# EPFL-IMOS/simple-SFOD

Measured on AMD Instinct MI355X. Metric: teacher+student train images/s on 1024x2048 synthetic, higher is better.
Workload: dtype bf16x3

## Files before the change

include/sfod_hip.h:

```cpp
#ifndef SFOD_HIP_H
#define SFOD_HIP_H
#include <stdint.h>
#ifdef __cplusplus
extern "C" {
#endif

#define SFOD_F32 0
#define SFOD_BF16 1
#define SFOD_BF16X3 2
#define SFOD_F16X3 3

int sfod_version(void);
const char* sfod_last_error(void);

int sfod_preprocess(const void* const* img_ptrs, const int32_t* sizes, int B, int Hp, int Wp,
                    int Cpad, const float* mean3, const float* std3, void* out, int dt,
                    void* stream);

int sfod_hflip_u8(const void* src, void* dst, int C, int H, int W, void* stream);

int sfod_resize_bilinear_u8(const void* src, void* dst, int C, int H, int W, int h, int w,
                            const int32_t* hbounds, const int32_t* hcoef, int ksize_h,
                            const int32_t* vbounds, const int32_t* vcoef, int ksize_v, int flip,
                            void* stream);
int sfod_resize_bilinear_u8_opt(const void* src, void* dst, int C, int H, int W, int y0, int x0, int ch, int cw,
                                int h, int w, const int32_t* hbounds, const int32_t* hcoef, int ksize_h,
                                const int32_t* vbounds, const int32_t* vcoef, int ksize_v, int flip_mode,
                                void* stream);

int sfod_mosaic_u8(const void* const* tiles, const void* const* tabs, const int32_t* geom, int n_tiles, int fill,
                   void* out, int H0, int W0, void* stream);

int sfod_conv_fwd(const void* x, const void* w, const float* bias, void* y, int B, int H, int W,
                  int Cin, int Cout, int ksize, int ldy, int act, float* stats, int dt, int out_dt,
                  void* stream);
int sfod_conv_fwd_ws(const void* x, const void* w, const uint32_t* w_absmax, const float* bias, void* y, int B, int H,
                     int W, int Cin, int Cout, int ksize, int ldy, int act, float* stats, int dt, int out_dt,
                     void* stream);
int64_t sfod_conv_fwd_scratch_bytes(int B, int H, int W, int Cin, int Cout, int ksize, int dt, int out_dt, int with_stats);
int sfod_conv_fwd_scratch(const void* x, const void* w, const uint32_t* w_absmax, const float* bias, void* y, int B, int H,
                          int W, int Cin, int Cout, int ksize, int ldy, int act, float* stats, int dt, int out_dt,
                          void* scratch, int64_t scratch_bytes, void* stream);
int sfod_conv_stats_blocks(int B, int H, int W, int Cin, int Cout, int ksize, int dt);
int sfod_set_conv_algo(int algo);
int sfod_conv_dgrad_bnred_blocks(int B, int H, int W, int Cin, int Cout, int dt);
int sfod_conv_dgrad_bnred(const void* x, const void* w, void* dz, int B, int H, int W, int Cin, int Cout, int dt,
                          const float* y, const float* mean, const float* invstd, const float* gamma,
                          const float* beta, float* red_ws, void* stream);
int sfod_conv_fwd_bnin_supported(int B, int H, int W, int Cin, int Cout, int dt);
int sfod_conv_fwd_bnin(const float* x_pre, const float* in_mean, const float* in_invstd, const float* in_gamma,
                       const float* in_beta, const void* w, const float* bias, float* y, int B, int H, int W, int Cin,
                       int Cout, int ldy, int act, float* stats, int dt, void* stream);
int sfod_set_gemm_tile(int tile);
int sfod_set_conv3x3_variant(int variant);
int sfod_last_conv_kernel(char* buf, int n);
int sfod_set_deterministic(int on);
int sfod_get_deterministic(void);
int sfod_set_conv3x3_m16(int on);
int sfod_set_wgrad3x3_pipe(int on);
int sfod_conv_fwd_algo(int B, int H, int W, int Cin, int Cout, int ksize, int dt);

int sfod_conv_first_supported(int B, int H, int W, int Cin, int Cout, int dt, int ldy);
int sfod_conv_first_fused(const void* x, const void* w, const float* bias, const float* scale,
                          const float* shift, void* y, float* stats, int B, int H, int W, int ldy,
                          int act, int dt, void* stream);
int sfod_conv_first_fused_ws(const void* x, const void* w, const uint32_t* w_absmax, const float* bias,
                             const float* scale, const float* shift, void* y, float* stats, int B, int H, int W,
                             int ldy, int act, int dt, void* stream);
int sfod_conv_first_stats_blocks(int B, int H, int W);
int sfod_set_conv_first_pipe(int on);
int sfod_set_conv_first_grid(int n);
int sfod_conv_first_bn_apply_supported(int B, int H, int W, int Cin, int Cout, int pool_flags, int dt, int y_dt);
int sfod_conv_first_bn_apply(const void* x, const void* w, const float* bias, const float* mean, const float* invstd,
                             const float* gamma, const float* beta, void* z, int B, int H, int W, int ldz, int dt,
                             void* stream);
int sfod_set_first_apply_recompute(int on);

int64_t sfod_conv_wgrad_ws_bytes(int B, int H, int W, int Cin, int Cout, int ksize, int lddy, int dt);
int sfod_conv_wgrad(const void* x, const void* dy, float* dw, int B, int H, int W, int Cin,
                    int Cout, int ksize, int lddy, int dt, void* ws, int64_t ws_bytes, void* stream);
int sfod_conv_wgrad_oihw_supported(int B, int H, int W, int Cin, int Cout, int ksize, int lddy, int dt);
int sfod_conv_wgrad_oihw(const void* x, const void* dy, float* dw_oihw, int B, int H, int W, int Cin,
                         int Cout, int ksize, int lddy, int dt, int accumulate, void* ws,
                         int64_t ws_bytes, void* stream);
int sfod_conv_first_wgrad_bn_supported(int B, int H, int W, int Cin, int Cout, int pool, int dt, int y_dt);
int sfod_conv_first_wgrad_bn(const void* x, const void* dz, const void* y, const float* mean, const float* invstd,
                             const float* gamma, const float* beta, const float* dgamma, const float* dbeta,
                             float* dw, int B, int H, int W, int Cin, int Cout, int dt, int oihw, int accumulate,
                             void* ws, int64_t ws_bytes, void* stream);
int sfod_set_first_wgrad_fused(int on);

int sfod_pack_conv_weight(const float* w_oihw, void* w_packed, int Cout, int Cin, int ksize,
                          int CinPad, int rot180, int dt, void* stream);
int sfod_pack_conv_weight_ws(const float* w_oihw, void* w_packed, uint32_t* absmax, int Cout, int Cin, int ksize,
                             int CinPad, int rot180, int dt, void* stream);
int sfod_pack_conv_weights_blocks(int Cout, int Cin, int ksize, int innerPad, int rot180);
int sfod_pack_conv_weights_multi(const int64_t* desc, int n, int total_blocks, int dt, void* stream);
int sfod_pack_conv_weights_multi_ws(const int64_t* desc, int n, int total_blocks, int dt, uint32_t* absmax ,
                                    void* stream);
int sfod_unpack_conv_wgrad(const float* dw_packed, float* dw_oihw, int Cout, int Cin, int ksize,
                           int CinPad, int accumulate, void* stream);
int sfod_pack_fc_weight(const float* w, void* out, int N, int K, int chw_c, int transpose, int dt,
                        void* stream);
int sfod_unpack_fc_wgrad(const float* dw_packed, float* dw, int N, int K, int chw_c,
                         int accumulate, void* stream);
int sfod_pack_fc_weight_ld(const float* w, void* out, int N, int K, int chw_c, int transpose, int ld,
                           int dt, void* stream);
int sfod_pack_fc_weight_ld_ws(const float* w, void* out, uint32_t* absmax, int N, int K, int chw_c, int transpose,
                              int ld, int dt, void* stream);
int sfod_unpack_fc_wgrad_ld(const float* dw_packed, float* dw, int N, int K, int chw_c, int ld,
                            int accumulate, void* stream);
int sfod_bias_grad(const void* dy, float* db, int M, int N, int ld, int accumulate, int dt,
                   void* stream);

int sfod_bn_finalize(const float* stats, int nblocks, int M, int C,
                     float* mean, float* invstd, float* running_mean, float* running_var,
                     float momentum, float eps, int update_running, int64_t* num_batches_tracked,
                     float* ws, void* stream);
int sfod_bn_finalize_pop(const float* stats, int nblocks, int M, int C,
                         float* mean, float* invstd, float* running_mean, float* running_var,
                         float momentum, float eps, int update_running, int64_t* num_batches_tracked,
                         float* ws, double* pop, int64_t pop_stride, void* stream);
int sfod_bn_pop_commit(const double* pop, int64_t pop_stride, const int64_t* table, const int64_t* table_host, int n,
                       void* stream);
int sfod_bn_pop_merge(double* dst, const double* src, int64_t columns, void* stream);
int sfod_set_bn_finalize_fused(int on);
int sfod_bn_finalize_ws_floats(int C);
int sfod_bn_relu_pool_fwd(const void* y, const float* mean, const float* invstd,
                          const float* gamma, const float* beta, void* z, int B, int H, int W,
                          int C, int pool, int dt, int out_dt, void* stream);
int sfod_bn_relu_pool_fwd2(const void* y, const float* mean, const float* invstd,
                           const float* gamma, const float* beta, void* z, void* z2, int B, int H, int W,
                           int C, int pool, int dt, int out_dt, void* stream);
int sfod_bn_add_relu_fwd(const void* y, const float* mean, const float* invstd, const float* gamma,
                         const float* beta, const void* residual, void* z, void* z_pairs, void* z_pairs2, int64_t rows,
                         int C, int dt, int pairs_dt, void* stream);
int sfod_bn_relu_pool_bwd(const void* dz, const void* y, const float* mean, const float* invstd,
                          const float* gamma, const float* beta, void* dy, float* dgamma,
                          float* dbeta, float* dgamma_acc, float* dbeta_acc, float* ws, int B, int H,
                          int W, int C, int pool, int dt, int out_dt, int reduced_blocks, void* stream);
#define SFOD_BN_BWD_SCRATCH_ROWS 32
int sfod_bn_bwd_ws_floats(int M, int C);
// ... 218 lines not shown
```

simple-sfod_amd/csrc/conv_internal.h:

```cpp
#pragma once
#include "common.h"

struct P3Plan {
  int ok;
  int G;
  int FM;
  int TH, TW;
  int tiles_y, tiles_x, tiles_n;
  int nblk;
  int m16;
};
P3Plan sfod_p3_plan(int B, int H, int W, int Cin, int Cout, int pairs = 0);
struct P3BnRed {
  const float* y;
  const float* mean;
  const float* invstd;
  const float* gamma;
  const float* beta;
  float* ws;
};
struct P3BnIn {
  const float* mean;
  const float* invstd;
  const float* gamma;
  const float* beta;
};
bool sfod_p3_bnin_ok(const P3Plan& p, int Cin_phys, int split);
int sfod_p3_launch(const P3Plan& p, const void* x, const void* w, const float* bias, void* y, float* stats,
                   int B, int H, int W, int Cin, int Cout, int ldy, int act, int out_f32, hipStream_t s, int split = 0,
                   const P3BnRed* red = nullptr, const unsigned* wamax = nullptr, const P3BnIn* bnin = nullptr);


struct W3Plan {
  int ok;
  int CO;
  int TH, TW, tiles_y, tiles_x;
  int co_tiles, ci_tiles;
  int tiles_per_split, nsplit, nslab;
  int64_t ws_bytes;
  int w64;
};
W3Plan sfod_w3_plan(int B, int H, int W, int Cin, int Cout, int lddy, int split = 0);
int sfod_w3_launch(const W3Plan& p, const void* x, const void* dy, float* dw, void* ws, int B, int H, int W,
                   int Cin, int Cout, int lddy, int out_mode, hipStream_t s, int split = 0);

struct W3BnApply {
  const float* dz;
  const float* y;
  const float* mean;
  const float* invstd;
  const float* gamma;
  const float* beta;
  const float* dgamma;
  const float* dbeta;
};
bool sfod_w3_bn_ok(const W3Plan& p, int Cin, int Cout);
int sfod_w3_bn_launch(const W3Plan& p, const void* x, const W3BnApply& bn, float* dw, void* ws, int B, int H, int W,
                      int out_mode, hipStream_t s);

bool sfod_deterministic();

void sfod_f16_poll_elementwise(unsigned* out, hipStream_t s);
void sfod_f16_poll_roi(unsigned* out, hipStream_t s);
void sfod_f16_poll_first(unsigned* out, hipStream_t s);
void sfod_f16_poll_stem(unsigned* out, hipStream_t s);
void sfod_f16_poll_gn(unsigned* out, hipStream_t s);
void sfod_f16_poll_cda(unsigned* out, hipStream_t s);

int sfod_f1_nblk(int B, int H, int W);
bool sfod_f1_bn_ok(int W);
struct F1BnApply {
  const float* mean;
  const float* invstd;
  const float* gamma;
  const float* beta;
};
int sfod_f1_launch(const void* x, const void* w, const float* bias, void* y, float* stats, int B, int H, int W,
                   int ldy, int act, hipStream_t s, const float* scale = nullptr, const float* shift = nullptr, int split = 0,
                   const unsigned* wamax = nullptr, const F1BnApply* bn = nullptr);
```

simple-sfod_amd/csrc/gemm_conv.hip:

```cpp
#include "conv_internal.h"
#include <algorithm>

typedef __attribute__((ext_vector_type(8))) __bf16 bf16x8;
typedef __attribute__((ext_vector_type(4))) short s16x4;
typedef __attribute__((ext_vector_type(8))) short s16x8;
typedef __attribute__((ext_vector_type(16))) float f32x16;
typedef __attribute__((ext_vector_type(4))) float f32x4;

#define LDS_PTR(p) ((__attribute__((address_space(3))) void*)(p))
#define GLB_PTR(p) ((const __attribute__((address_space(1))) void*)(p))

__device__ __attribute__((aligned(16))) unsigned int g_zero_page[64];

struct ConvArgs {
  int M;
  int H, W;
  int Cin;
  int Cout;
  int ks;
  int cpt_shift;
  int kchunks;
  int ldy;
  int act;
  const unsigned* wamax;
  int kt_per;
  int nsplit;
  int64_t slab;
};

template <typename T> struct Chunk { static constexpr int E = 16 / sizeof(T); };

__device__ __forceinline__ void glds16(const void* g, void* l) {
  __builtin_amdgcn_global_load_lds(GLB_PTR(g), LDS_PTR(l), 16, 0, 0);
}

__device__ __forceinline__ void chunk_to_tap(int gq, int ks, int cpt_shift, int& tap, int& cc) {
  if (ks == 1) { tap = 0; cc = gq; }
  else { tap = gq >> cpt_shift; cc = gq & ((1 << cpt_shift) - 1); }
}

__device__ __forceinline__ float apply_act(float v, int act) {
  const float slope = (act == 2) ? 0.2f : 1.f;
  return fmaxf(v, (act == 1) ? 0.f : v * slope);
}

template <typename T, typename OutT, int WM, int WN, bool UT, int WR, int NST, int SPLIT = 0, int BKB = 128>
__global__ void __launch_bounds__(WR * 128)
k_conv_fwd(const T* __restrict__ x, const T* __restrict__ w, const float* __restrict__ bias,
           OutT* __restrict__ y, float* __restrict__ stats, ConvArgs a, int tiles_n, int ntiles) {
  static_assert(WM == 2, "wave tile is 64 rows");
  constexpr int NT = WR * 128;
  constexpr int BM = WR * 32 * WM, BN = 64 * WN;
  constexpr int E = Chunk<T>::E;
  constexpr int CPR = BKB / 16;
  constexpr int RPI = 1024 / BKB;
  constexpr int STAGE = (BM + BN) * BKB;
  static_assert(BKB == 128 || BKB == 64, "LDS rows of 128 or 64 bytes");
  extern __shared__ __attribute__((aligned(16))) unsigned char smem[];
  auto swz = [](int r) { return BKB == 128 ? ((r >> 1) & 7) : ((r >> 2) & 3); };

  int bid = blockIdx.x;
  {
    const int q = ntiles / 8, r = ntiles % 8, xcd = bid % 8;
    bid = (xcd < r ? xcd * (q + 1) : r * (q + 1) + (xcd - r) * q) + bid / 8;
  }
  const int tile_n = bid % tiles_n, tile_m = bid / tiles_n;
  const int m0 = tile_m * BM, n0 = tile_n * BN;
  const int lane = threadIdx.x & 63, wave = threadIdx.x >> 6;
  const int wr = wave >> 1, wc = wave & 1;
  const int taps = a.ks * a.ks;
  const int HW = a.H * a.W;

  constexpr int AI = BM / (RPI * 2 * WR), BI = BN / (RPI * 2 * WR);
  static_assert(BI >= 1, "tile too narrow for this wave count");
  int a_row[AI];
  int a_oy[AI], a_ox[AI];
  int64_t a_pix[AI];
  for (int i = 0; i < AI; ++i) {
    const int q = wave * AI + i;
    const int row = q * RPI + lane / CPR;
    a_row[i] = row;
    const int m = m0 + row;
    if (m < a.M) {
      const int rem = m % HW;
// ... 901 lines not shown
          }
#pragma unroll
          for (int j = 0; j < WN; ++j) {
            const int col = wc * 32 * WN + j * 32 + (g16 & 1) * 16 + 4 * tp;
            const s16x4 v = __builtin_amdgcn_ds_read_tr16_b64_v4i16(
                (__attribute__((address_space(3))) s16x4*)LDS_PTR(sB + prow * RB + ((col * 2) ^ sw)));
            bfr[j][4 * e + 0] = v[0]; bfr[j][4 * e + 1] = v[1]; bfr[j][4 * e + 2] = v[2]; bfr[j][4 * e + 3] = v[3];
          }
        }
#pragma unroll
        for (int i = 0; i < WM; ++i)
#pragma unroll
          for (int j = 0; j < WN; ++j)
            acc[i][j] = __builtin_amdgcn_mfma_f32_32x32x16_bf16(
                __builtin_bit_cast(bf16x8, af[i]), __builtin_bit_cast(bf16x8, bfr[j]), acc[i][j], 0, 0, 0);
      }
    } else {
#pragma unroll 4
      for (int s = 0; s < BKP / 2; ++s) {
        const int prow = 2 * s + h;
        float af[WM], bfr[WN];
#pragma unroll
        for (int i = 0; i < WM; ++i)
          af[i] = *reinterpret_cast<const float*>(sA + prow * RA + (wr * 32 * WM + i * 32 + (lane & 31)) * 4);
#pragma unroll
        for (int j = 0; j < WN; ++j)
          bfr[j] = *reinterpret_cast<const float*>(sB + prow * RB + (wc * 32 * WN + j * 32 + (lane & 31)) * 4);
#pragma unroll
        for (int i = 0; i < WM; ++i)
#pragma unroll
          for (int j = 0; j < WN; ++j)
            acc[i][j] = __builtin_amdgcn_mfma_f32_32x32x2f32(af[i], bfr[j], acc[i][j], 0, 0, 0);
      }
    }
  };

  const int KT = (p_end - p_begin + BKP - 1) / BKP;
  stage_load(0, 0);
  asm volatile("s_waitcnt vmcnt(0)" ::: "memory");
  __syncthreads();
  int cur = 0;
  for (int kt = 0; kt < KT - 1; ++kt) {
    stage_load(kt + 1, cur ^ 1);
    stage_compute(cur);
    asm volatile("s_waitcnt vmcnt(0)" ::: "memory");
    __syncthreads();
    cur ^= 1;
  }
  stage_compute(cur);

  if constexpr (SPLIT) {
    __syncthreads();
    float* red = reinterpret_cast<float*>(smem);
#pragma unroll
    for (int i = 0; i < 2; ++i)
#pragma unroll
      for (int j = 0; j < 2; ++j)
#pragma unroll
        for (int r = 0; r < 16; ++r) red[((wave * 4 + i * 2 + j) * 16 + r) * 64 + lane] = acc[i][j][r];
    __syncthreads();
    for (int e = threadIdx.x; e < 4096; e += 256) {
      const float v = (red[e] + red[4096 + e]) + (red[8192 + e] + red[12288 + e]);
      const int ln = e & 63, r = (e >> 6) & 15, t = e >> 10;
      const int co = co0 + (t >> 1) * 32 + (r & 3) + 8 * (r >> 2) + 4 * (ln >> 5);
      const int n = n0 + (t & 1) * 32 + (ln & 31);
      if (co < a.Cout && n < a.Ntot) wg_emit(dw, a, split, co, n, v);
    }
    return;
  }
#pragma unroll
  for (int i = 0; i < WM; ++i)
#pragma unroll
    for (int j = 0; j < WN; ++j) {
      const int n = n0 + wc * 32 * WN + j * 32 + (lane & 31);
#pragma unroll
      for (int r = 0; r < 16; ++r) {
        const int co = co0 + wr * 32 * WM + i * 32 + (r & 3) + 8 * (r >> 2) + 4 * h;
        if (co < a.Cout && n < a.Ntot) wg_emit(dw, a, split, co, n, acc[i][j][r]);
      }
    }
}


__global__ void __launch_bounds__(512)
k_conv_wgrad_x3w(const bf16_t* __restrict__ x, const bf16_t* __restrict__ dy, float* __restrict__ dw, WgradArgs a) {
  constexpr int BM = 128, BN = 256, BKP = 32;
  constexpr int RA = BM * 4, RB = BN * 4;
  constexpr int TA = BKP * RA, TB = BKP * RB, STAGE = TA + TB;
  constexpr int AI = TA / 1024 / 8, BI = TB / 1024 / 8;
  extern __shared__ __attribute__((aligned(16))) unsigned char smem[];
  const int lane = threadIdx.x & 63, wave = threadIdx.x >> 6;
  const int wr = wave >> 2, wc = wave & 3;
  int bid = blockIdx.x;
  {
    const int nt = gridDim.x, q = nt / 8, r = nt % 8, xcd = bid % 8;
    bid = (xcd < r ? xcd * (q + 1) : r * (q + 1) + (xcd - r) * q) + bid / 8;
  }
  const int tiles = a.tiles_n * a.tiles_m;
  const int split = bid / tiles, trem = bid % tiles;
  const int n0 = (trem / a.tiles_m) * BN, co0 = (trem % a.tiles_m) * BM;
  const int p_begin = split * a.pix_per_split;
  const int p_end = min(a.M, p_begin + a.pix_per_split);
  if (p_begin >= p_end) return;
  const int taps = a.ks * a.ks;

  int a_prow[AI], a_goff[AI];
  bool a_ok[AI];
  for (int i = 0; i < AI; ++i) {
    const int o = (wave * AI + i) * 1024 + lane * 16;
    const int prow = o / RA, pcol = (o % RA) >> 4;
    const int lc = pcol ^ ((prow & 3) << 2);
    const int col = co0 + (lc & 15) * 8;
    a_prow[i] = prow;
    a_goff[i] = col * 2 + (lc >> 4) * 8;
    a_ok[i] = (col + 8 <= a.lddy) && (col < a.Cout);
  }
  int b_prow[BI], b_tap[BI], b_cc[BI], b_oy[BI], b_ox[BI];
  bool b_ok[BI];
  for (int i = 0; i < BI; ++i) {
    const int o = (wave * BI + i) * 1024 + lane * 16;
    const int prow = o / RB, pcol = (o % RB) >> 4;
    const int lc = pcol ^ ((prow & 3) << 2);
    const int nq = n0 / 8 + (lc & 31);
    int tap, cc;
    chunk_to_tap(nq, a.ks, a.cpt_shift, tap, cc);
    b_prow[i] = prow;
    b_tap[i] = tap;
    b_cc[i] = cc * 2 + (lc >> 5);
    b_ok[i] = (nq < a.nchunks) && (tap < taps);
    const int rem = (p_begin + prow) % (a.H * a.W);
    b_oy[i] = rem / a.W;
    b_ox[i] = rem % a.W;
  }

  auto stage_load = [&](int kt, int buf) {
    unsigned char* sA = smem + buf * STAGE;
    unsigned char* sB = sA + TA;
    const int pbase = p_begin + kt * BKP;
#pragma unroll
    for (int i = 0; i < AI; ++i) {
      const int pix = pbase + a_prow[i];
      const void* src = (pix < p_end && a_ok[i]) ? (const void*)(dy + (int64_t)pix * a.lddy * 2 + a_goff[i])
                                                 : (const void*)g_zero_page;
      glds16(src, sA + (wave * AI + i) * 1024);
    }
#pragma unroll
    for (int i = 0; i < BI; ++i) {
      const int pix = pbase + b_prow[i];
      const void* src = g_zero_page;
      if (pix < p_end && b_ok[i]) {
        if (a.ks == 1) {
          src = x + (int64_t)pix * a.Cin * 2 + (int64_t)b_cc[i] * 8;
        } else {
          const int ky = b_tap[i] / 3, kx = b_tap[i] - ky * 3;
          const int iy = b_oy[i] + ky - 1, ix = b_ox[i] + kx - 1;
          if (iy >= 0 && iy < a.H && ix >= 0 && ix < a.W)
            src = x + ((int64_t)pix + (int64_t)(ky - 1) * a.W + (kx - 1)) * a.Cin * 2 + (int64_t)b_cc[i] * 8;
        }
      }
      glds16(src, sB + (wave * BI + i) * 1024);
      if (a.ks != 1) {
        b_ox[i] += BKP;
        while (b_ox[i] >= a.W) {
          b_ox[i] -= a.W;
          if (++b_oy[i] == a.H) b_oy[i] = 0;
        }
      }
    }
  };

  f32x16 acc[2][2];
  for (int i = 0; i < 2; ++i)
    for (int j = 0; j < 2; ++j)
      for (int r = 0; r < 16; ++r) acc[i][j][r] = 0.f;
  const int h = lane >> 5;
  const int g16 = lane >> 4, t16 = lane & 15;
  const int tq = t16 >> 2, tp = t16 & 3;

  auto stage_compute = [&](int buf) {
    const unsigned char* sA = smem + buf * STAGE;
    const unsigned char* sB = sA + TA;
#pragma unroll
    for (int s = 0; s < BKP / 16; ++s) {
      s16x8 ah[2], al[2], bh[2], bl[2];
#pragma unroll
      for (int e = 0; e < 2; ++e) {
        const int prow = 16 * s + 8 * h + 4 * e + tq;
        const int sw = (prow & 3) << 6;
#pragma unroll
        for (int f = 0; f < 2; ++f) {
          const int ca = (wr * 64 + f * 32 + (g16 & 1) * 16 + 4 * tp) * 2;
          const int cb = (wc * 64 + f * 32 + (g16 & 1) * 16 + 4 * tp) * 2;
          const s16x4 v0 = __builtin_amdgcn_ds_read_tr16_b64_v4i16((__attribute__((address_space(3))) s16x4*)LDS_PTR(sA + prow * RA + (ca ^ sw)));
          const s16x4 v1 = __builtin_amdgcn_ds_read_tr16_b64_v4i16((__attribute__((address_space(3))) s16x4*)LDS_PTR(sA + prow * RA + ((ca + RA / 2) ^ sw)));
          const s16x4 v2 = __builtin_amdgcn_ds_read_tr16_b64_v4i16((__attribute__((address_space(3))) s16x4*)LDS_PTR(sB + prow * RB + (cb ^ sw)));
          const s16x4 v3 = __builtin_amdgcn_ds_read_tr16_b64_v4i16((__attribute__((address_space(3))) s16x4*)LDS_PTR(sB + prow * RB + ((cb + RB / 2) ^ sw)));
#pragma unroll
          for (int k = 0; k < 4; ++k) {
            ah[f][4 * e + k] = v0[k]; al[f][4 * e + k] = v1[k];
            bh[f][4 * e + k] = v2[k]; bl[f][4 * e + k] = v3[k];
          }
        }
      }
#pragma unroll
      for (int i = 0; i < 2; ++i)
#pragma unroll
        for (int j = 0; j < 2; ++j)
          acc[i][j] = __builtin_amdgcn_mfma_f32_32x32x16_bf16(__builtin_bit_cast(bf16x8, ah[i]), __builtin_bit_cast(bf16x8, bl[j]), acc[i][j], 0, 0, 0);
#pragma unroll
      for (int i = 0; i < 2; ++i)
#pragma unroll
        for (int j = 0; j < 2; ++j)
          acc[i][j] = __builtin_amdgcn_mfma_f32_32x32x16_bf16(__builtin_bit_cast(bf16x8, al[i]), __builtin_bit_cast(bf16x8, bh[j]), acc[i][j], 0, 0, 0);
#pragma unroll
      for (int i = 0; i < 2; ++i)
#pragma unroll
        for (int j = 0; j < 2; ++j)
          acc[i][j] = __builtin_amdgcn_mfma_f32_32x32x16_bf16(__builtin_bit_cast(bf16x8, ah[i]), __builtin_bit_cast(bf16x8, bh[j]), acc[i][j], 0, 0, 0);
    }
  };

  const int KT = (p_end - p_begin + BKP - 1) / BKP;
  stage_load(0, 0);
  if (KT > 1) stage_load(1, 1);
  int cur = 0, nxt = 2;
  for (int kt = 0; kt < KT; ++kt) {
    if (kt + 1 < KT) asm volatile("s_waitcnt vmcnt(%0) lgkmcnt(0)" ::"n"(AI + BI) : "memory");
    else asm volatile("s_waitcnt vmcnt(0) lgkmcnt(0)" ::: "memory");
    __builtin_amdgcn_s_barrier();
    asm volatile("" ::: "memory");
    if (kt + 2 < KT) stage_load(kt + 2, nxt);
    stage_compute(cur);
    cur = (cur == 2) ? 0 : cur + 1;
    nxt = (nxt == 2) ? 0 : nxt + 1;
  }
#pragma unroll
  for (int i = 0; i < 2; ++i)
#pragma unroll
    for (int j = 0; j < 2; ++j) {
      const int n = n0 + wc * 64 + j * 32 + (lane & 31);
#pragma unroll
      for (int r = 0; r < 16; ++r) {
        const int co = co0 + wr * 64 + i * 32 + (r & 3) + 8 * (r >> 2) + 4 * h;
        if (co < a.Cout && n < a.Ntot) wg_emit(dw, a, split, co, n, acc[i][j][r]);
      }
    }
}

static SfodKnob g_deterministic{"SFOD_DETERMINISTIC", 0, sfod_knob_bool};
extern "C" int sfod_set_deterministic(int on) { g_deterministic.set(on); return 0; }
bool sfod_deterministic() { return g_deterministic.get() != 0; }
extern "C" int sfod_get_deterministic(void) { return sfod_deterministic() ? 1 : 0; }

__global__ void __launch_bounds__(256) k_wgrad_slab_sum(const float* __restrict__ ws, float* __restrict__ dw, int64_t n,
                                                       int nslab, int64_t stride) {
  for (int64_t i = ((int64_t)blockIdx.x * 256 + threadIdx.x) * 4; i < n; i += (int64_t)gridDim.x * 1024) {
    if (i + 4 <= n && (stride & 3) == 0) {
      float4 acc = *reinterpret_cast<const float4*>(dw + i);
      for (int sl = 0; sl < nslab; ++sl) {
        const float4 v = *reinterpret_cast<const float4*>(ws + sl * stride + i);
        acc.x += v.x; acc.y += v.y; acc.z += v.z; acc.w += v.w;
      }
      *reinterpret_cast<float4*>(dw + i) = acc;
    } else {
      for (int64_t e = i; e < n && e < i + 4; ++e) {
        float acc = dw[e];
        for (int sl = 0; sl < nslab; ++sl) acc += ws[sl * stride + e];
        dw[e] = acc;
      }
    }
  }
}

enum WgradTile { WGRAD_TILE_AUTO, WGRAD_TILE_64, WGRAD_TILE_WIDE };
struct GenWgradPlan { int wide, tiles_n, tiles_m, splits, pps; };
static GenWgradPlan gen_wgrad_plan(int M, int Cout, int Ntot, int dt, WgradTile force) {
  GenWgradPlan g;
  const int split = (dt == SFOD_BF16X3);
  g.wide = split && Cout >= 128 && Ntot >= 256 && force != WGRAD_TILE_64 &&
           (force == WGRAD_TILE_WIDE || (int64_t)((Ntot + 255) / 256) * ((Cout + 127) / 128) >= 256);
  if (g.wide) {
    constexpr int BKP = 32;
    g.tiles_n = (Ntot + 255) / 256; g.tiles_m = (Cout + 127) / 128;
    const int tiles = g.tiles_n * g.tiles_m;
    const int max_splits = std::max(1, M / (8 * BKP));
    int best = 1;
    double best_eff = 0.0;
    for (int sp = 1; sp <= std::min(max_splits, 512); ++sp) {
      const int64_t wgs = (int64_t)tiles * sp;
      const double eff = (double)wgs / (double)((wgs + 255) / 256 * 256);
      if (eff > best_eff + 1e-9) { best_eff = eff; best = sp; }
      if (eff >= 0.85 && wgs >= 512) { best = sp; break; }
      if (wgs >= 4096) break;
    }
    int pps = (M + best - 1) / best;
    pps = (pps + BKP - 1) / BKP * BKP;
    g.pps = pps;
    g.splits = (M + pps - 1) / pps;
    return g;
  }
  const int BKP = (dt == SFOD_F32) ? 32 : 64;
  const int TILE = split ? 64 : 128;
  g.tiles_n = (Ntot + TILE - 1) / TILE; g.tiles_m = (Cout + TILE - 1) / TILE;
  int splits = (1024 + g.tiles_n * g.tiles_m - 1) / (g.tiles_n * g.tiles_m);
  const int max_splits = (M + BKP - 1) / BKP;
  if (splits > max_splits) splits = max_splits;
  if (splits < 1) splits = 1;
  int pps = (M + splits - 1) / splits;
  pps = (pps + BKP - 1) / BKP * BKP;
  g.pps = pps;
  g.splits = (M + pps - 1) / pps;
  return g;
}

enum WgradKind { WGRAD_NONE, WGRAD_PATCH, WGRAD_GEMM, WGRAD_GEMM_WIDE };
// ... 25 lines not shown
      p.first_bn_ok = split && nb == B && lddy == Cout && sfod_w3_bn_ok(full, Cin, Cout);
      return p;
    }
  }
  p.force = (algo == 3) ? WGRAD_TILE_64 : (algo == 4 ? WGRAD_TILE_WIDE : WGRAD_TILE_AUTO);
  p.gen = gen_wgrad_plan(M, Cout, Ntot, dt, p.force);
  p.kind = p.gen.wide ? WGRAD_GEMM_WIDE : WGRAD_GEMM;
  if (ksize == 3) p.cpt_shift = ilog2_exact(Cin / (dt == SFOD_F32 ? 4 : 8));
  p.slabs = sfod_deterministic() && p.gen.splits > 1;
  if (p.slabs) p.ws_bytes = (int64_t)p.gen.splits * Cout * Ntot * 4;
  return p;
}

extern "C" int64_t sfod_conv_wgrad_ws_bytes(int B, int H, int W, int Cin, int Cout, int ksize, int lddy, int dt) {
  return conv_wgrad_plan(B, H, W, Cin, Cout, ksize, lddy, dt).ws_bytes;
}

extern "C" int sfod_conv_wgrad_oihw_supported(int B, int H, int W, int Cin, int Cout, int ksize, int lddy, int dt) {
  return conv_wgrad_plan(B, H, W, Cin, Cout, ksize, lddy, dt).kind == WGRAD_PATCH ? 1 : 0;
}

static int wgrad_patch_launch(const ConvWgradPlan& p, const void* x, const void* dy, float* dw, void* ws, int64_t ws_bytes,
                              int B, int H, int W, int Cin, int Cout, int lddy, int dt, int out_mode, hipStream_t s) {
  if (ws == nullptr || ws_bytes < p.ws_bytes) {
    sfod_set_error("wgrad: workspace too small (sfod_conv_wgrad_ws_bytes)");
    return SFOD_EBADARG;
  }
  const int split = (dt == SFOD_BF16X3);
  const int64_t eb = split ? 4 : 2;
  for (int b0 = 0; b0 < B; b0 += p.nb) {
    const int n = std::min(p.nb, B - b0);
    const char* xb = (const char*)x + (int64_t)b0 * H * W * Cin * eb;
    const char* dyb = (const char*)dy + (int64_t)b0 * H * W * lddy * eb;
    const int mode = (b0 == 0) ? out_mode : (out_mode == 1 ? 2 : out_mode);
    const int rc = sfod_w3_launch(n == p.nb ? p.full : p.rest, xb, dyb, dw, ws, n, H, W, Cin, Cout, lddy, mode, s, split);
    if (rc) return rc;
  }
  return 0;
}

extern "C" int sfod_conv_wgrad_oihw(const void* x, const void* dy, float* dw_oihw, int B, int H, int W, int Cin,
                                    int Cout, int ksize, int lddy, int dt, int accumulate, void* ws,
                                    int64_t ws_bytes, void* stream) {
  sfod_note_conv_kernel(nullptr);
  SFOD_REQUIRE(conv_shape_fits(B, H, W, Cin, Cout, ksize) && sfod_ints_ok({lddy}) && sfod_i64s_ok({ws_bytes}),
               "conv_wgrad_oihw: negative or oversized extent");
  SFOD_REQUIRE(x != nullptr && dy != nullptr && dw_oihw != nullptr, "conv_wgrad_oihw: null operand");
  SFOD_REQUIRE(lddy >= Cout, "conv_wgrad_oihw: lddy < Cout");
  const ConvWgradPlan p = conv_wgrad_plan(B, H, W, Cin, Cout, ksize, lddy, dt);
  SFOD_REQUIRE(p.kind == WGRAD_PATCH,
               "wgrad_oihw: shape not served by the halo-patch kernel (query sfod_conv_wgrad_oihw_supported)");
  return wgrad_patch_launch(p, x, dy, dw_oihw, ws, ws_bytes, B, H, W, Cin, Cout, lddy, dt, accumulate ? 2 : 1,
                            (hipStream_t)stream);
}

static SfodKnob g_first_wgrad_fused{"SFOD_FIRST_WGRAD_FUSED", 1, sfod_knob_bool};
extern "C" int sfod_set_first_wgrad_fused(int on) { g_first_wgrad_fused.set(on); return 0; }

extern "C" int sfod_conv_first_wgrad_bn_supported(int B, int H, int W, int Cin, int Cout, int pool, int dt, int y_dt) {
  if (g_first_wgrad_fused.get() == 0 || pool != 0 || y_dt != SFOD_F32) return 0;
  return conv_wgrad_plan(B, H, W, Cin, Cout, 3, Cout, dt).first_bn_ok ? 1 : 0;
}

extern "C" int sfod_conv_first_wgrad_bn(const void* x, const void* dz, const void* y, const float* mean,
                                        const float* invstd, const float* gamma, const float* beta,
                                        const float* dgamma, const float* dbeta, float* dw, int B, int H, int W,
                                        int Cin, int Cout, int dt, int oihw, int accumulate, void* ws,
                                        int64_t ws_bytes, void* stream) {
  sfod_note_conv_kernel(nullptr);
  SFOD_REQUIRE(conv_shape_fits(B, H, W, Cin, Cout, 3) && sfod_i64s_ok({ws_bytes}),
               "conv_first_wgrad_bn: negative or oversized extent");
  SFOD_REQUIRE(x != nullptr && dz != nullptr && y != nullptr && dw != nullptr, "conv_first_wgrad_bn: null operand");
  SFOD_REQUIRE(mean && invstd && gamma && beta && dgamma && dbeta, "conv_first_wgrad_bn: null BatchNorm argument");
  const ConvWgradPlan p = conv_wgrad_plan(B, H, W, Cin, Cout, 3, Cout, dt);
  SFOD_REQUIRE(p.first_bn_ok, "conv_first_wgrad_bn: shape not served (query sfod_conv_first_wgrad_bn_supported)");
  SFOD_REQUIRE(ws != nullptr && ws_bytes >= p.ws_bytes, "conv_first_wgrad_bn: workspace too small (sfod_conv_wgrad_ws_bytes)");
  W3BnApply bn;
  bn.dz = (const float*)dz; bn.y = (const float*)y; bn.mean = mean; bn.invstd = invstd; bn.gamma = gamma; bn.beta = beta;
  bn.dgamma = dgamma; bn.dbeta = dbeta;
  const int out_mode = oihw ? (accumulate ? 2 : 1) : 0;
  return sfod_w3_bn_launch(p.full, x, bn, dw, ws, B, H, W, out_mode, (hipStream_t)stream);
}

static int wgrad_gemm_launch(const ConvWgradPlan& p, const void* x, const void* dy, float* dw, void* ws, int64_t ws_bytes,
                             int B, int H, int W, int Cin, int Cout, int ksize, int lddy, int dt, hipStream_t s) {
  SFOD_REQUIRE(p.cpt_shift >= 0, "wgrad3x3: Cin/chunk must be a power of two");
  if (p.slabs && (ws == nullptr || ws_bytes < p.ws_bytes)) {
    sfod_set_error("wgrad: deterministic mode needs the workspace of sfod_conv_wgrad_ws_bytes");
    return SFOD_EBADARG;
  }
  const GenWgradPlan& g = p.gen;
  WgradArgs a;
  a.M = B * H * W; a.H = H; a.W = W; a.Cin = Cin; a.Cout = Cout; a.ks = ksize; a.lddy = lddy;
  a.cpt_shift = p.cpt_shift;
  a.nchunks = ksize * ksize * (Cin / (dt == SFOD_F32 ? 4 : 8));
  a.Ntot = ksize * ksize * Cin;
  a.pix_per_split = g.pps;
  a.tiles_n = g.tiles_n;
  a.tiles_m = g.tiles_m;
  a.slab_stride = p.slabs ? (int64_t)Cout * a.Ntot : 0;
  float* dw_out = p.slabs ? (float*)ws : dw;
  struct { const void* fn; const char* name; int threads, lds; } k;
  if (p.kind == WGRAD_GEMM_WIDE) {
    k = {(const void*)k_conv_wgrad_x3w, "k_conv_wgrad_x3w", 512, 3 * 32 * (128 + 256) * 4};
    static const hipError_t attr_rc = hipFuncSetAttribute(k.fn, hipFuncAttributeMaxDynamicSharedMemorySize, k.lds);
    SFOD_REQUIRE(attr_rc == hipSuccess, "wgrad: cannot raise the dynamic LDS limit");
  } else if (dt == SFOD_F32) {
    k = {(const void*)k_conv_wgrad<float, 2, 2>, "k_conv_wgrad<float,2,2,0>", 256, 2 * 2 * 32 * 512};
  } else if (dt == SFOD_BF16X3) {
    k = {(const void*)k_conv_wgrad<bf16_t, 2, 2, true>, "k_conv_wgrad<bf16_t,2,2,1>", 256, 2 * 2 * 64 * 256};
  } else {
    k = {(const void*)k_conv_wgrad<bf16_t, 2, 2>, "k_conv_wgrad<bf16_t,2,2,0>", 256, 2 * 2 * 64 * 256};
  }
  sfod_note_conv_kernel(k.name);
  void* args[] = {(void*)&x, (void*)&dy, (void*)&dw_out, (void*)&a};
  (void)hipLaunchKernel(k.fn, dim3(g.tiles_n * g.tiles_m * g.splits), dim3(k.threads), args, k.lds, s);
  int rc = sfod_check_launch(p.kind == WGRAD_GEMM_WIDE ? "conv_wgrad_x3w" : "conv_wgrad");
  if (rc == 0 && p.slabs) {
    const int64_t n = (int64_t)Cout * a.Ntot;
    hipLaunchKernelGGL(k_wgrad_slab_sum, dim3(cdiv(n, 1024) > 4096 ? 4096 : cdiv(n, 1024)), dim3(256), 0, s,
                       (const float*)ws, dw, n, g.splits, a.slab_stride);
    rc = sfod_check_launch("wgrad_slab_sum");
  }
  return rc;
}

extern "C" int sfod_conv_wgrad(const void* x, const void* dy, float* dw, int B, int H, int W, int Cin,
                               int Cout, int ksize, int lddy, int dt, void* ws, int64_t ws_bytes,
                               void* stream) {
  sfod_note_conv_kernel(nullptr);
  SFOD_REQUIRE(conv_shape_fits(B, H, W, Cin, Cout, ksize) && sfod_ints_ok({lddy}) && sfod_i64s_ok({ws_bytes}),
               "conv_wgrad: negative or oversized extent");
  SFOD_REQUIRE(x != nullptr && dy != nullptr && dw != nullptr, "conv_wgrad: null operand");
  SFOD_REQUIRE(lddy >= Cout, "conv_wgrad: lddy < Cout");
  SFOD_REQUIRE(ksize == 1 || ksize == 3, "wgrad: ksize must be 1 or 3");
  SFOD_REQUIRE(dt == SFOD_F32 || dt == SFOD_BF16 || dt == SFOD_BF16X3, "wgrad: unknown dt");
  const int E = (dt == SFOD_F32) ? 4 : 8;
  SFOD_REQUIRE(Cin % E == 0 && lddy % E == 0, "wgrad: Cin / lddy must be multiples of the 16-byte chunk (bf16x3: of 8)");
  if ((int64_t)B * H * W == 0) return 0;
  SFOD_REQUIRE(dt != SFOD_BF16X3 || Cout % 8 == 0, "wgrad: bf16x3 needs Cout % 8 == 0");
  const ConvWgradPlan p = conv_wgrad_plan(B, H, W, Cin, Cout, ksize, lddy, dt);
  hipStream_t s = (hipStream_t)stream;
  if (p.kind == WGRAD_NONE) return 0;
  if (p.kind == WGRAD_PATCH) return wgrad_patch_launch(p, x, dy, dw, ws, ws_bytes, B, H, W, Cin, Cout, lddy, dt, 0, s);
  return wgrad_gemm_launch(p, x, dy, dw, ws, ws_bytes, B, H, W, Cin, Cout, ksize, lddy, dt, s);
}
```

simple-sfod_amd/csrc/wgrad3x3_patch.hip:

```cpp
#include "conv_internal.h"
#include <type_traits>
#include <stdlib.h>

typedef __attribute__((ext_vector_type(8))) __bf16 bf16x8;
typedef __attribute__((ext_vector_type(4))) short s16x4;
typedef __attribute__((ext_vector_type(8))) short s16x8;
typedef __attribute__((ext_vector_type(16))) float f32x16;

#define LDS_PTR(p) ((__attribute__((address_space(3))) void*)(p))

namespace {

template <int J> using IC = std::integral_constant<int, J>;

constexpr int XROWS = 384;
constexpr int XPLANE = XROWS * 64;
constexpr int XBUF = 2 * XPLANE;
constexpr int DY_OFF = 2 * XBUF;
constexpr int DYSLOT = 4 * 64 * 64;
constexpr int TAB_OFF = DY_OFF + 3 * DYSLOT;
constexpr int TABP_OFF = TAB_OFF;
constexpr int TABT_OFF = TAB_OFF + 512;
constexpr int TABR_OFF = TAB_OFF + 1024;
constexpr int TABX_OFF = TAB_OFF + 1024 + 768;
constexpr int TABD_OFF = TABX_OFF + 1536;
constexpr int LDS_TOTAL = TABD_OFF + 1024;
constexpr unsigned OOB_OFF = 0x80000000u;

struct W3Args {
  const bf16_t* x;
  const bf16_t* dy;
  float* slab;
  int B, H, W, Cin, Cout, lddy;
  int TH, TW, PW;
  int tiles_y, tiles_x;
  int ntiles;
  int tiles_per_split;
  int co_tiles, ci_tiles, nsplit;
};

__device__ __forceinline__ void bufload16(__amdgpu_buffer_rsrc_t rsrc, unsigned voff, unsigned soff, void* l) {
  __builtin_amdgcn_raw_ptr_buffer_load_lds(rsrc, LDS_PTR(l), 16, (int)voff, (int)soff, 0, 0);
}
template <int N> __device__ __forceinline__ void wait_vm() {
  asm volatile("s_waitcnt vmcnt(%0)" ::"n"(N) : "memory");
}
template <int OFF> __device__ __forceinline__ s16x4 tr_read(unsigned addr) {
  s16x4 v;
  asm volatile("ds_read_b64_tr_b16 %0, %1 offset:%2" : "=v"(v) : "v"(addr), "n"(OFF));
  return v;
}
template <int N> __device__ __forceinline__ void wait_lgkm() {
  asm volatile("s_waitcnt lgkmcnt(%0)" ::"n"(N) : "memory");
  __builtin_amdgcn_sched_barrier(0);
}
__device__ __forceinline__ bf16x8 cat8(s16x4 a, s16x4 b) {
  return __builtin_bit_cast(bf16x8, __builtin_shufflevector(a, b, 0, 1, 2, 3, 4, 5, 6, 7));
}

template <int CO, bool SPLIT = false, bool PIPE = false>
__global__ void __launch_bounds__(512)
k_wgrad3x3_patch(W3Args a) {
  static_assert(!SPLIT || CO == 4, "bf16x3 operands use the four-plane dy ring");
  static_assert(!PIPE || SPLIT, "the pipelined chunk loop exists for the bf16x3 variant");
  constexpr int ND = CO / 2;
  constexpr int KG = SPLIT ? 4 : ((CO == 4) ? 1 : 2);
  constexpr int KS = 4 / KG;
  constexpr int EB = SPLIT ? 4 : 2;
  constexpr int CO_TILE = SPLIT ? 64 : CO * 32, CI_TILE = SPLIT ? 32 : 64;
  extern __shared__ __attribute__((aligned(16))) unsigned char smem[];
  const int lane = threadIdx.x & 63;
  const int wave = __builtin_amdgcn_readfirstlane(threadIdx.x >> 6);
  const int wco = SPLIT ? (wave & 1) : ((CO == 4) ? (wave >> 1) : ((wave >> 1) & 1));
  const int wci = SPLIT ? 0 : (wave & 1);
  const int kg = SPLIT ? (wave >> 1) : ((CO == 4) ? 0 : (wave >> 2));
  const int h = lane >> 5, g1 = (lane >> 4) & 1, t16 = lane & 15;
  const int tq = t16 >> 2, tp = t16 & 3;

  int bid = blockIdx.x;
  {
    const int nt = gridDim.x, q = nt / 8, r = nt % 8, xcd = bid % 8;
    bid = (xcd < r ? xcd * (q + 1) : r * (q + 1) + (xcd - r) * q) + bid / 8;
  }
  const int pairs = a.co_tiles * a.ci_tiles;
  const int split = bid / pairs;
  const int pr = bid - split * pairs;
  const int co0 = (pr / a.ci_tiles) * CO_TILE, ci0 = (pr % a.ci_tiles) * CI_TILE;
  const int t_begin = split * a.tiles_per_split;
  const int t_end = min(a.ntiles, t_begin + a.tiles_per_split);
  const int PW = a.PW;
  const int npix = a.TH * a.TW;

  unsigned short* tabP = reinterpret_cast<unsigned short*>(smem + TABP_OFF);
  unsigned short* tabT = reinterpret_cast<unsigned short*>(smem + TABT_OFF);
  unsigned short* tabR = reinterpret_cast<unsigned short*>(smem + TABR_OFF);
  if (threadIdx.x < 256) {
    const int p = threadIdx.x;
    if (p < npix) {
      const int ty = p / a.TW, tx = p - ty * a.TW;
      tabP[p] = (unsigned short)(ty * PW + tx);
      tabT[p] = (unsigned short)((ty << 8) | tx);
    } else {
      tabP[p] = 0;
      tabT[p] = 0xffff;
    }
  }
  if (threadIdx.x < XROWS) {
    const int r = threadIdx.x;
    const int py = r / PW, px = r - py * PW;
    tabR[r] = (py < a.TH + 2) ? (unsigned short)((py << 8) | px) : (unsigned short)0xffff;
  }
  __syncthreads();

  const __amdgpu_buffer_rsrc_t xres = __builtin_amdgcn_make_buffer_rsrc(
      (void*)a.x, (short)0, (int)min((int64_t)0x7fffffff, (int64_t)a.B * a.H * a.W * a.Cin * EB), 0x00020000);
  const __amdgpu_buffer_rsrc_t dres = __builtin_amdgcn_make_buffer_rsrc(
      (void*)a.dy, (short)0, (int)min((int64_t)0x7fffffff, (int64_t)a.B * a.H * a.W * a.lddy * EB), 0x00020000);

  int pr_col;
  {
    const int plane = wave >> 2;
    if constexpr (SPLIT) {
      const int c = ci0 + (lane & 3) * 8;
      pr_col = (c < a.Cin) ? (c * 4 + plane * 16) : -1;
    } else {
      const int c = ci0 + plane * 32 + (lane & 3) * 8;
      pr_col = (c < a.Cin) ? c * 2 : -1;
    }
  }
  auto patch_row = [&](int k) { return (int)tabR[((wave * 6 + k) % 24) * 16 + (lane >> 2)]; };
  int dy_col;
  {
    const int q = wave * ND;
    if constexpr (SPLIT) {
      const int pl = q >> 2;
      const int c = co0 + (pl >> 1) * 32 + (lane & 3) * 8;
      dy_col = (c + 8 <= a.lddy && c < a.Cout) ? (c * 4 + (pl & 1) * 16) : -1;
// ... 1042 lines not shown
```

simple-sfod_amd/native.py:

```python
import collections
import ctypes
import math
import os
import re
import warnings

import torch

warnings.filterwarnings("ignore", message="ComplexHalf support is experimental")

_HERE = os.path.dirname(os.path.abspath(__file__))
HEADER = os.path.join(os.path.dirname(_HERE), "include", "sfod_hip.h")
SO_PATH = os.environ.get("SFOD_HIP_LIB", os.path.join(_HERE, "lib", "libsfod_hip.so"))

F32, BF16, BF16X3, F16X3 = 0, 1, 2, 3

SPLIT_DTYPE = torch.complex32
SPLITH_DTYPE = torch.uint32
PAIR_DTYPES = (SPLIT_DTYPE, SPLITH_DTYPE)

COMPUTE_MODES = {"fp32": F32, "bf16": BF16, "bf16x3": BF16X3, "f16x3": F16X3}


def mode_dt(name):
# ... 148 lines not shown
    return e << (n - 1).bit_length()


def pad_channels(x, cp):
    c = x.shape[-1]
    if cp == c:
        return x
    raw = torch.int32 if x.dtype in PAIR_DTYPES else x.dtype
    out = torch.zeros(*x.shape[:-1], cp, dtype=raw, device=x.device)
    out[..., :c] = x.view(raw)
    return out.view(x.dtype)


def operands_for(t, dtype, need_grad):
    gdt = grad_dtype_of(dtype)
    if not need_grad:
        return as_operand(t, dtype), None
    if gdt == dtype:
        op = as_operand(t, dtype)
        return op, op
    if t.dtype == torch.float32 and dtype == SPLITH_DTYPE and gdt == SPLIT_DTYPE:
        t = t.contiguous()
        a = torch.empty(t.shape, dtype=SPLITH_DTYPE, device=t.device)
        b = torch.empty(t.shape, dtype=SPLIT_DTYPE, device=t.device)
        call("sfod_cast_pairs_both", t, a, b, t.numel())
        return a, b
    return as_operand(t, dtype), as_operand(t, gdt)


class _Everything:
    def __contains__(self, item):
        return True


class KernelTimer:

    def __init__(self, watch=("sfod_conv_fwd", "sfod_conv_wgrad", "sfod_conv_wgrad_oihw")):
        self.watch = _Everything() if watch is None else set(watch)
        self.records = []

    def summary(self):
        torch.cuda.synchronize()
        out = {}
        for name, flops, a, b in self.records:
            d = out.setdefault(name, {"launches": 0, "ms": 0.0, "flops": 0.0})
            d["launches"] += 1
            d["ms"] += a.elapsed_time(b)
            d["flops"] += flops
        return out


_timer = None


def set_timer(timer):
    global _timer
    _timer = timer


def call(name, *args, timer_name=None, flops=0.0, tag=""):
    lib = load()
    conv = [(_p(a) if isinstance(a, torch.Tensor) else a) for a in args]
    if _timer is not None and (timer_name or name) in _timer.watch:
        a, b = torch.cuda.Event(enable_timing=True), torch.cuda.Event(enable_timing=True)
        a.record()
        rc = getattr(lib, name)(*conv, _stream())
        b.record()
        _timer.records.append(((timer_name or name) + tag, flops, a, b))
    else:
        rc = getattr(lib, name)(*conv, _stream())
    _chk(rc, name)


def query(name, *args):
    return getattr(load(), name)(*args)


def set_conv_algo(algo):
    load().sfod_set_conv_algo(int(algo))


def set_wgrad3x3_pipe(on):
    load().sfod_set_wgrad3x3_pipe(int(on))


def set_gemm_tile(tile):
    load().sfod_set_gemm_tile(int(tile))


def set_conv3x3_variant(variant):
    load().sfod_set_conv3x3_variant(int(variant))


def last_conv_kernel():
    buf = ctypes.create_string_buffer(256)
    n = load().sfod_last_conv_kernel(buf, len(buf))
    if n < 0:
        _chk(n, "sfod_last_conv_kernel")
    return buf.value.decode()


def set_deterministic(on):
    lib = load()
    prev = bool(lib.sfod_get_deterministic())
    lib.sfod_set_deterministic(int(bool(on)))
    return prev


def set_bn_finalize_fused(on):
    load().sfod_set_bn_finalize_fused(int(bool(on)))


def set_conv3x3_m16(on):
    load().sfod_set_conv3x3_m16(int(on))


_const_cache = {}


def dev_const(values, dtype, device):
    key = (values, dtype, str(device))
    t = _const_cache.get(key)
    if t is None:
        if len(_const_cache) > 4096:
            _const_cache.clear()
        t = torch.tensor(values, dtype=dtype).to(device)
        _const_cache[key] = t
    return t


_PIN_SLOTS, _PIN_WIDTH = 32, 64
_pin_ring = {}


def _pinned_upload_i64(values, dev):
    n = len(values)
    if n > _PIN_WIDTH:
        return torch.tensor(values, dtype=torch.int64).to(dev)
    st = _pin_ring.get(dev)
    if st is None:
        st = {"buf": torch.empty(_PIN_SLOTS, _PIN_WIDTH, dtype=torch.int64).pin_memory(), "ev": [None] * _PIN_SLOTS,
              "next": 0}
        _pin_ring[dev] = st
    i = st["next"]
    st["next"] = (i + 1) % _PIN_SLOTS
    if st["ev"][i] is not None:
        st["ev"][i].synchronize()
    slot = st["buf"][i, :n]
    slot.copy_(torch.tensor(values, dtype=torch.int64))
    out = slot.to(dev, non_blocking=True)
    ev = torch.cuda.Event()
    ev.record()
    st["ev"][i] = ev
    return out


def preprocess(images_u8, Hp, Wp, cpad, mean, std, dt):
    dev = images_u8[0].device
    B = len(images_u8)
    imgs = [im.contiguous() for im in images_u8]
    ptrs = _pinned_upload_i64([im.data_ptr() for im in imgs], dev)
    sizes = dev_const(tuple((int(im.shape[1]), int(im.shape[2])) for im in imgs), torch.int32, dev)
    out = torch.empty(B, Hp, Wp, cpad, dtype=torch_dtype(dt), device=dev)
    m = (ctypes.c_float * 3)(*mean)
    s = (ctypes.c_float * 3)(*std)
    lib = load()
# ... 1269 lines not shown
```

Before: 164.6.

## Software-pipeline LDS transpose reads with MFMA in wide bf16x3 wgrad kernel

```diff
diff --git a/include/sfod_hip.h b/include/sfod_hip.h
--- a/include/sfod_hip.h
+++ b/include/sfod_hip.h
@@ -58,6 +58,7 @@
 int sfod_get_deterministic(void);
 int sfod_set_conv3x3_m16(int on);
 int sfod_set_wgrad3x3_pipe(int on);
+int sfod_set_wgrad_wide_pipe(int on);
 int sfod_conv_fwd_algo(int B, int H, int W, int Cin, int Cout, int ksize, int dt);
 
 int sfod_conv_first_supported(int B, int H, int W, int Cin, int Cout, int dt, int ldy);
diff --git a/simple-sfod_amd/csrc/conv_internal.h b/simple-sfod_amd/csrc/conv_internal.h
--- a/simple-sfod_amd/csrc/conv_internal.h
+++ b/simple-sfod_amd/csrc/conv_internal.h
@@ -1,5 +1,16 @@
 #pragma once
 #include "common.h"
+
+typedef __attribute__((ext_vector_type(4))) short s16x4;
+template <int OFF> __device__ __forceinline__ s16x4 tr_read(unsigned addr) {
+  s16x4 v;
+  asm volatile("ds_read_b64_tr_b16 %0, %1 offset:%2" : "=v"(v) : "v"(addr), "n"(OFF));
+  return v;
+}
+template <int N> __device__ __forceinline__ void wait_lgkm() {
+  asm volatile("s_waitcnt lgkmcnt(%0)" ::"n"(N) : "memory");
+  __builtin_amdgcn_sched_barrier(0);
+}
 
 struct P3Plan {
   int ok;
diff --git a/simple-sfod_amd/csrc/gemm_conv.hip b/simple-sfod_amd/csrc/gemm_conv.hip
--- a/simple-sfod_amd/csrc/gemm_conv.hip
+++ b/simple-sfod_amd/csrc/gemm_conv.hip
@@ -1,5 +1,6 @@
 #include "conv_internal.h"
 #include <algorithm>
+#include <type_traits>
 
 typedef __attribute__((ext_vector_type(8))) __bf16 bf16x8;
 typedef __attribute__((ext_vector_type(4))) short s16x4;
@@ -1067,6 +1068,10 @@
 }
 
 
+__device__ __forceinline__ bf16x8 x3w_cat8(s16x4 a, s16x4 b) {
+  return __builtin_bit_cast(bf16x8, __builtin_shufflevector(a, b, 0, 1, 2, 3, 4, 5, 6, 7));
+}
+template <bool LIN, bool PIPE>
 __global__ void __launch_bounds__(512)
 k_conv_wgrad_x3w(const bf16_t* __restrict__ x, const bf16_t* __restrict__ dy, float* __restrict__ dw, WgradArgs a) {
   constexpr int BM = 128, BN = 256, BKP = 32;
@@ -1091,6 +1096,7 @@
 
   int a_prow[AI], a_goff[AI];
   bool a_ok[AI];
+  const bf16_t* a_src[AI];
   for (int i = 0; i < AI; ++i) {
     const int o = (wave * AI + i) * 1024 + lane * 16;
     const int prow = o / RA, pcol = (o % RA) >> 4;
@@ -1099,9 +1105,11 @@
     a_prow[i] = prow;
     a_goff[i] = col * 2 + (lc >> 4) * 8;
     a_ok[i] = (col + 8 <= a.lddy) && (col < a.Cout);
+    a_src[i] = dy + (int64_t)(p_begin + prow) * a.lddy * 2 + a_goff[i];
   }
   int b_prow[BI], b_tap[BI], b_cc[BI], b_oy[BI], b_ox[BI];
   bool b_ok[BI];
+  const bf16_t* b_src[BI] = {};
   for (int i = 0; i < BI; ++i) {
     const int o = (wave * BI + i) * 1024 + lane * 16;
     const int prow = o / RB, pcol = (o % RB) >> 4;
@@ -1113,15 +1121,38 @@
     b_tap[i] = tap;
     b_cc[i] = cc * 2 + (lc >> 5);
     b_ok[i] = (nq < a.nchunks) && (tap < taps);
-    const int rem = (p_begin + prow) % (a.H * a.W);
-    b_oy[i] = rem / a.W;
-    b_ox[i] = rem % a.W;
-  }
+    if constexpr (LIN) {
+      b_src[i] = x + (int64_t)(p_begin + prow) * a.Cin * 2 + (int64_t)b_cc[i] * 8;
+      b_oy[i] = b_ox[i] = 0;
+    } else {
+      const int rem = (p_begin + prow) % (a.H * a.W);
+      b_oy[i] = rem / a.W;
+      b_ox[i] = rem % a.W;
+    }
+  }
+  const int64_t a_step = (int64_t)BKP * a.lddy * 2, b_step = (int64_t)BKP * a.Cin * 2;
 
   auto stage_load = [&](int kt, int buf) {
     unsigned char* sA = smem + buf * STAGE;
     unsigned char* sB = sA + TA;
     const int pbase = p_begin + kt * BKP;
+    if constexpr (LIN) {
+#pragma unroll
+      for (int i = 0; i < AI; ++i) {
+        const int pix = pbase + a_prow[i];
+        const void* src = (pix < p_end && a_ok[i]) ? (const void*)a_src[i] : (const void*)g_zero_page;
+        glds16(src, sA + (wave * AI + i) * 1024);
+        a_src[i] += a_step;
+      }
+#pragma unroll
+      for (int i = 0; i < BI; ++i) {
+        const int pix = pbase + b_prow[i];
+        const void* src = (pix < p_end && b_ok[i]) ? (const void*)b_src[i] : (const void*)g_zero_page;
+        glds16(src, sB + (wave * BI + i) * 1024);
+        b_src[i] += b_step;
+      }
+      return;
+    }
 #pragma unroll
     for (int i = 0; i < AI; ++i) {
       const int pix = pbase + a_prow[i];
@@ -1205,6 +1236,83 @@
     }
   };
 
+  unsigned fa[2], fb[2];
+  {
+    const unsigned lds0 = (unsigned)(uintptr_t)LDS_PTR(smem);
+    const int sw = tq << 6;
+#pragma unroll
+    for (int f = 0; f < 2; ++f) {
+      const int ca = (wr * 64 + f * 32 + (g16 & 1) * 16 + 4 * tp) * 2;
+      const int cb = (wc * 64 + f * 32 + (g16 & 1) * 16 + 4 * tp) * 2;
+      fa[f] = lds0 + (unsigned)((8 * h + tq) * RA + (ca ^ sw));
+      fb[f] = lds0 + (unsigned)(TA + (8 * h + tq) * RB + (cb ^ sw));
+    }
+  }
+  auto issue_hl = [&](auto S, s16x4* d, const unsigned* ra, const unsigned* rb) {
+    constexpr int OA = 16 * decltype(S)::value * RA, OB = 16 * decltype(S)::value * RB + RB / 2;
+#ifdef WGX3W_KO_READS
+    asm volatile("" : "+v"(d[0]), "+v"(d[1]), "+v"(d[2]), "+v"(d[3]), "+v"(d[4]), "+v"(d[5]), "+v"(d[6]), "+v"(d[7]));
+    (void)ra; (void)rb;
+    return;
+#endif
+    d[0] = tr_read<OA>(ra[0]); d[1] = tr_read<OA + 4 * RA>(ra[0]);
+    d[2] = tr_read<OA>(ra[1]); d[3] = tr_read<OA + 4 * RA>(ra[1]);
+    d[4] = tr_read<OB>(rb[0]); d[5] = tr_read<OB + 4 * RB>(rb[0]);
+    d[6] = tr_read<OB>(rb[1]); d[7] = tr_read<OB + 4 * RB>(rb[1]);
+  };
+  auto issue_lh = [&](auto S, s16x4* d, const unsigned* ra, const unsigned* rb) {
+    constexpr int OA = 16 * decltype(S)::value * RA + RA / 2, OB = 16 * decltype(S)::value * RB;
+#ifdef WGX3W_KO_READS
+    asm volatile("" : "+v"(d[0]), "+v"(d[1]), "+v"(d[2]), "+v"(d[3]), "+v"(d[4]), "+v"(d[5]), "+v"(d[6]), "+v"(d[7]));
+    (void)ra; (void)rb;
+    return;
+#endif
+    d[0] = tr_read<OA>(ra[0]); d[1] = tr_read<OA + 4 * RA>(ra[0]);
+    d[2] = tr_read<OA>(ra[1]); d[3] = tr_read<OA + 4 * RA>(ra[1]);
+    d[4] = tr_read<OB>(rb[0]); d[5] = tr_read<OB + 4 * RB>(rb[0]);
+    d[6] = tr_read<OB>(rb[1]); d[7] = tr_read<OB + 4 * RB>(rb[1]);
+  };
+  auto mfma4 = [&](const s16x4* da, const s16x4* db) {
+#pragma unroll
+    for (int i = 0; i < 2; ++i)
+#pragma unroll
+      for (int j = 0; j < 2; ++j) {
+#ifdef WGX3W_KO_MFMA
+        asm volatile("" ::"v"(da[2 * i]), "v"(da[2 * i + 1]), "v"(db[2 * j]), "v"(db[2 * j + 1]));
+        acc[i][j][0] += 1.0f;
+#else
+        acc[i][j] = __builtin_amdgcn_mfma_f32_32x32x16_bf16(x3w_cat8(da[2 * i], da[2 * i + 1]), x3w_cat8(db[2 * j], db[2 * j + 1]),
+                                                            acc[i][j], 0, 0, 0);
+#endif
+      }
+  };
+  auto stage_compute_pipe = [&](int buf, auto&& load) {
+    const unsigned sb = (unsigned)(buf * STAGE);
+    const unsigned ra[2] = {fa[0] + sb, fa[1] + sb}, rb[2] = {fb[0] + sb, fb[1] + sb};
+    using S0 = std::integral_constant<int, 0>;
+    using S1 = std::integral_constant<int, 1>;
+#ifdef WGX3W_KO_READS
+    s16x4 p[8] = {}, q[8] = {}, u[8] = {}, v[8] = {};
+#else
+    s16x4 p[8], q[8], u[8], v[8];
+#endif
+    issue_hl(S0{}, p, ra, rb);
+    issue_lh(S0{}, q, ra, rb);
+    load();
+    wait_lgkm<8>();
+    mfma4(p, p + 4);
+    issue_hl(S1{}, u, ra, rb);
+    wait_lgkm<8>();
+    mfma4(q, q + 4);
+    mfma4(p, q + 4);
+    issue_lh(S1{}, v, ra, rb);
+    wait_lgkm<8>();
+    mfma4(u, u + 4);
+    wait_lgkm<0>();
+    mfma4(v, v + 4);
+    mfma4(u, v + 4);
+  };
+
   const int KT = (p_end - p_begin + BKP - 1) / BKP;
   stage_load(0, 0);
   if (KT > 1) stage_load(1, 1);
@@ -1212,10 +1320,21 @@
   for (int kt = 0; kt < KT; ++kt) {
     if (kt + 1 < KT) asm volatile("s_waitcnt vmcnt(%0) lgkmcnt(0)" ::"n"(AI + BI) : "memory");
     else asm volatile("s_waitcnt vmcnt(0) lgkmcnt(0)" ::: "memory");
+#ifdef WGX3W_KO_BARRIER
+    if constexpr (!PIPE)
+#endif
     __builtin_amdgcn_s_barrier();
     asm volatile("" ::: "memory");
-    if (kt + 2 < KT) stage_load(kt + 2, nxt);
-    stage_compute(cur);
+    if constexpr (PIPE) {
+#ifdef WGX3W_KO_DMA
+      stage_compute_pipe(cur, [&]() {});
+#else
+      stage_compute_pipe(cur, [&]() { if (kt + 2 < KT) stage_load(kt + 2, nxt); });
+#endif
+    } else {
+      if (kt + 2 < KT) stage_load(kt + 2, nxt);
+      stage_compute(cur);
+    }
     cur = (cur == 2) ? 0 : cur + 1;
     nxt = (nxt == 2) ? 0 : nxt + 1;
   }
@@ -1407,6 +1526,9 @@
   return sfod_w3_bn_launch(p.full, x, bn, dw, ws, B, H, W, out_mode, (hipStream_t)stream);
 }
 
+static SfodKnob g_wgx3w_pipe{"SFOD_WGX3W_PIPE", 1, sfod_knob_bool};
+extern "C" int sfod_set_wgrad_wide_pipe(int on) { g_wgx3w_pipe.set(on); return 0; }
+
 static int wgrad_gemm_launch(const ConvWgradPlan& p, const void* x, const void* dy, float* dw, void* ws, int64_t ws_bytes,
                              int B, int H, int W, int Cin, int Cout, int ksize, int lddy, int dt, hipStream_t s) {
   SFOD_REQUIRE(p.cpt_shift >= 0, "wgrad3x3: Cin/chunk must be a power of two");
@@ -1427,8 +1549,18 @@
   float* dw_out = p.slabs ? (float*)ws : dw;
   struct { const void* fn; const char* name; int threads, lds; } k;
   if (p.kind == WGRAD_GEMM_WIDE) {
-    k = {(const void*)k_conv_wgrad_x3w, "k_conv_wgrad_x3w", 512, 3 * 32 * (128 + 256) * 4};
-    static const hipError_t attr_rc = hipFuncSetAttribute(k.fn, hipFuncAttributeMaxDynamicSharedMemorySize, k.lds);
+    const bool pipe = g_wgx3w_pipe.get() != 0;
+    const void* fn = !pipe ? (const void*)k_conv_wgrad_x3w<false, false>
+                           : (ksize == 1 ? (const void*)k_conv_wgrad_x3w<true, true> : (const void*)k_conv_wgrad_x3w<false, true>);
+    k = {fn, "k_conv_wgrad_x3w", 512, 3 * 32 * (128 + 256) * 4};
+    static const hipError_t attr_rc = [&]() {
+      for (const void* f : {(const void*)k_conv_wgrad_x3w<false, false>, (const void*)k_conv_wgrad_x3w<false, true>,
+                            (const void*)k_conv_wgrad_x3w<true, true>}) {
+        const hipError_t rc = hipFuncSetAttribute(f, hipFuncAttributeMaxDynamicSharedMemorySize, k.lds);
+        if (rc != hipSuccess) return rc;
+      }
+      return hipSuccess;
+    }();
     SFOD_REQUIRE(attr_rc == hipSuccess, "wgrad: cannot raise the dynamic LDS limit");
   } else if (dt == SFOD_F32) {
     k = {(const void*)k_conv_wgrad<float, 2, 2>, "k_conv_wgrad<float,2,2,0>", 256, 2 * 2 * 32 * 512};
diff --git a/simple-sfod_amd/csrc/wgrad3x3_patch.hip b/simple-sfod_amd/csrc/wgrad3x3_patch.hip
--- a/simple-sfod_amd/csrc/wgrad3x3_patch.hip
+++ b/simple-sfod_amd/csrc/wgrad3x3_patch.hip
@@ -44,15 +44,6 @@
 }
 template <int N> __device__ __forceinline__ void wait_vm() {
   asm volatile("s_waitcnt vmcnt(%0)" ::"n"(N) : "memory");
-}
-template <int OFF> __device__ __forceinline__ s16x4 tr_read(unsigned addr) {
-  s16x4 v;
-  asm volatile("ds_read_b64_tr_b16 %0, %1 offset:%2" : "=v"(v) : "v"(addr), "n"(OFF));
-  return v;
-}
-template <int N> __device__ __forceinline__ void wait_lgkm() {
-  asm volatile("s_waitcnt lgkmcnt(%0)" ::"n"(N) : "memory");
-  __builtin_amdgcn_sched_barrier(0);
 }
 __device__ __forceinline__ bf16x8 cat8(s16x4 a, s16x4 b) {
   return __builtin_bit_cast(bf16x8, __builtin_shufflevector(a, b, 0, 1, 2, 3, 4, 5, 6, 7));
diff --git a/simple-sfod_amd/native.py b/simple-sfod_amd/native.py
--- a/simple-sfod_amd/native.py
+++ b/simple-sfod_amd/native.py
@@ -254,6 +254,10 @@
 
 def set_wgrad3x3_pipe(on):
     load().sfod_set_wgrad3x3_pipe(int(on))
+
+
+def set_wgrad_wide_pipe(on):
+    load().sfod_set_wgrad_wide_pipe(int(on))
 
 
 def set_gemm_tile(tile):
```

After: 165.8 (median of 6 runs). No clear change (+0.7%).
